# szbonaldo/FedMLP

Measured on AMD Instinct MI355X. Metric: images/sec/client (ICH 224x224 bs=128) at 1/2/4/8 GPUs; mAP vs ref, higher is better.
Workload: dtype f32; 1 GPU; FedMLP stage1 step, Resnet18, ICH-shaped synthetic 3x224x224, C=5, bs=128, one client per GPU, FedAvg all-reduce every 40 steps + once at end; parallelism=clients1, rccl_ranks=1, stream_mode=default: frozen teacher + weight gradients on the engine's side stream, arithmetic=fp32 operands+sums; products as 6 exact bf16 partials on the bf16 matrix pipe

## Files before the change

fedmlp_amd/_lib.py:

```python
import ctypes as C
import os

_HERE = os.path.dirname(os.path.abspath(__file__))
LIB_PATH = os.environ.get("FEDMLP_HIP_LIB") or os.path.join(_HERE, "libfedmlp_hip.so")

FM_MAX_CLASSES = 32
FM_COMM_ID_BYTES = 128


class FmConfig(C.Structure):
    _fields_ = [("model", C.c_int32), ("n_classes", C.c_int32), ("in_h", C.c_int32),
                ("in_w", C.c_int32), ("max_images", C.c_int32), ("reserved", C.c_int32 * 3),
                ("stream", C.c_void_p)]


class FmAdam(C.Structure):
    _fields_ = [("lr", C.c_float), ("beta1", C.c_float), ("beta2", C.c_float),
                ("eps", C.c_float), ("weight_decay", C.c_float)]


class FmSgd(C.Structure):
    _fields_ = [("lr", C.c_float), ("momentum", C.c_float), ("dampening", C.c_float),
                ("weight_decay", C.c_float), ("nesterov", C.c_int32)]

# ... 63 lines not shown
    "fm_profile_read": (C.c_int, [_P, _I32, C.POINTER(_I64), C.POINTER(C.c_double),
                                  C.POINTER(C.c_double)]),
    "fm_comm_preflight": (C.c_int, []),
    "fm_comm_unique_id": (C.c_int, [C.POINTER(C.c_uint8)]),
    "fm_comm_init": (C.c_int, [_P, C.POINTER(C.c_uint8), _I32, _I32]),
    "fm_comm_destroy": (C.c_int, [_P]),
    "fm_comm_size": (C.c_int, [_P]),
    "fm_fedavg_allreduce": (C.c_int, [_P, C.c_float]),
    "fm_fedavg_tao": (C.c_int, [_P, C.POINTER(C.c_double), C.c_double, _F, C.POINTER(C.c_double)]),
    "fm_fedavg_proto": (C.c_int, [_P, _P, C.c_double, _F, _P]),
    "fm_profile_ops": (C.c_int, [_P, _I32, C.c_char_p, _I32]),
    "fm_debug_num_convs": (C.c_int, [_P]),
    "fm_debug_conv_info": (C.c_int, [_P, _I32, C.POINTER(_I32)]),
    "fm_debug_conv": (C.c_int, [_P, _I32, _I32, _P, _P, _P, _I32, _I32, _P]),
    "fm_debug_block_dgrad": (C.c_int, [_P, _I32, _P, _P, _P, _I32]),
    "fm_debug_pw": (C.c_int, [_P, _I32, _I32, _P, _P, _P, _I32, _I32, _P, _P, _P, _P]),
    "fm_debug_proj_bwd": (C.c_int, [_P, _I32, _I32, _P, _P, _P, _P, _P, _I32, _I32, _P, _P]),
    "fm_debug_exp_bwd": (C.c_int, [_P, _I32, _P, _P, _P, _P, _P, _I32, _I32, _P, _P]),
    "fm_debug_get_grads": (C.c_int, [_P, _P]),
    "fm_debug_activation": (C.c_int, [_P, _I32, _I32, _I32, _P, C.POINTER(_I32)]),
    "fm_debug_stem_masks": (C.c_int, [_P, _I32, _I32, _P, _P]),
    "fm_debug_lose_part": (C.c_int, [_I32]),
    "fm_debug_ew": (C.c_int, [_P, _I32, C.POINTER(_P), C.POINTER(_I32), _F]),
    "fm_debug_eff": (C.c_int, [_P, _I32, C.POINTER(_P), C.POINTER(_I32), _F]),
    "fm_debug_eff_ws": (C.c_int, [_I32, C.POINTER(_I32), C.POINTER(C.c_int64)]),
}

_lib = None


# ... 39 lines not shown
```

fedmlp_amd/csrc/common.h:

```cpp
#pragma once
#include <hip/hip_runtime.h>
#include <stdint.h>

#include <stdlib.h>

typedef float f32x4 __attribute__((ext_vector_type(4)));

#ifndef FM_F32_FAST_SWISH
#define FM_F32_FAST_SWISH 1
#endif
#ifdef __HIPCC__
__device__ __forceinline__ float fm_swish_f32(float v)
{
#if FM_F32_FAST_SWISH
    return v * __builtin_amdgcn_rcpf(1.f + __expf(-v));
#else
    return v / (1.f + expf(-v));
#endif
}
#endif


#ifndef FM_MFMA_SPLIT_DEFAULT
#define FM_MFMA_SPLIT_DEFAULT 6
// ... 51 lines not shown
template <int NV> __device__ __forceinline__ void ldf(const float* p, f32x4 (&v)[NV])
{
#pragma unroll
    for (int h = 0; h < NV; ++h) v[h] = ld4(p + 4 * h);
}
#endif

#define PCONV_MAX_JOBS 5
struct PconvJob {
    int ntaps;
    unsigned long long tapcode;
    int cib, icc2;
    unsigned wofs, wofs2;
    int Hg, Wg;
    int oh0, ow0;
    int nsteps, k2;
    int npix;
    float rcpHW, rcpW;
    int tilesN;
    int tile0, step0;
};
inline unsigned long long pconv_tapcode(const int* dh, const int* dw, int ntaps)
{
    unsigned long long c = 0;
    for (int t = 0; t < ntaps; ++t) c |= (unsigned long long)(((dh[t] + 1) & 3) | (((dw[t] + 1) & 3) << 2)) << (4 * t);
    return c;
}

struct IgemmParams {
    const float* W;
// ... 119 lines not shown
```

fedmlp_amd/csrc/engine.hip:

```cpp
#include <math.h>
#include <stdio.h>
#include <string.h>

#include <algorithm>
#include <string>
#include <vector>

#include "../../include/fedmlp_hip.h"
#include "../../include/fedmlp_hip_debug.h"
#include "comm.h"
#include "common.h"
#include "kernels.h"
#include "pwconv.h"

static thread_local std::string g_err;
const char* fm_last_error(void) { return g_err.c_str(); }
const char* fm_version(void) { return "fedmlp_hip 0.2 (gfx950)"; }

#define HIPCHK(x)                                                                              \
    do {                                                                                       \
        hipError_t e_ = (x);                                                                   \
        if (e_ != hipSuccess) {                                                                \
            char b_[512];                                                                      \
            snprintf(b_, sizeof b_, "%s:%d %s -> %s", __FILE__, __LINE__, #x, hipGetErrorString(e_)); \
// ... 144 lines not shown
    size_t off_fcw = 0, off_fcb = 0, off_gamma = 0, off_beta = 0, off_rm = 0, off_rv = 0;
    int64_t nf_sd = 0, ni_sd = 0;
    float *grad = nullptr, *adam_m = nullptr, *adam_v = nullptr;
    float* stage_sd = nullptr;
    fm_adam hp{3e-5f, 0.9f, 0.999f, 1e-8f, 5e-4f};
    int64_t adam_t = 0;
    float *x4 = nullptr, *dyh0 = nullptr;
    float* x3 = nullptr;
    bool stem_rows = false;
    unsigned short* x3p = nullptr;
    long long x3p_plane_elems = 0;
    uint8_t* idx0 = nullptr;
    float *GA = nullptr, *GB = nullptr, *GC = nullptr, *GD = nullptr, *GE = nullptr;
    float *ws_stats = nullptr, *ws_part = nullptr;
    int stats_conv = -1, stats_tiles_n = 0;
    size_t slab_floats = 0;
    float *ca = nullptr, *cb = nullptr, *cc = nullptr;
    float *feat = nullptr, *logits = nullptr, *tfeat = nullptr, *tlogits = nullptr, *dlogits = nullptr;
    float* psum = nullptr;
    int64_t *pcnt = nullptr, *tcnt = nullptr;
    float* zeros = nullptr;
    int *sel_counts = nullptr, *sel_top = nullptr, *sel_bot = nullptr, *cls_dev = nullptr;
    int sel_cap = 0;
    int* tag_buf = nullptr;
    size_t tag_buf_ints = 0;
    bool prof = false, prof_fail = false;
    hipError_t soft_err = hipSuccess;
    int* dev_err = nullptr;
    int* host_err = nullptr;
    int* host_err_dev = nullptr;
// ... 651 lines not shown
    bool side = e->stream_mode != 1;
    const Conv& c0 = e->convs[0];
    if (e->model == 0) {
        const size_t pooled = B * (c0.hout / 2) * (c0.wout / 2) * 64;
        DALLOC(e->idx0, pooled);
        DALLOC(e->dyh0, B * c0.hout * c0.wout * 64);
        DALLOC(e->GA, pooled); DALLOC(e->GB, pooled); DALLOC(e->GC, pooled); DALLOC(e->GD, pooled); DALLOC(e->GE, pooled);
    } else {
        const EffSizes z = eff_sizes(e);
        AALLOC(e->GA, z.g_io); AALLOC(e->GB, z.g_io);
        AALLOC(e->T_small, z.t_small); AALLOC(e->T_big, z.t_big);
        DALLOC(e->se_dgp, B * z.max_ce); DALLOC(e->se_drp, B * z.max_cs); DALLOC(e->se_ds, B * z.max_ce);
        side = side && side_fits(e);
        DALLOC(e->hfeat, B * e->D);
    }
    DALLOC(e->ws_stats, max_stats);
    DALLOC(e->ws_part, (size_t)2 * (1024 + 32) * 2 * e->maxC);
    e->slab_floats = std::max<size_t>(max_slab * 8, (size_t)48 << 20);
    DALLOC(e->main.ws_slab, e->slab_floats);
    e->main.rec = e->main.ws_slab;
    DALLOC(e->ca, 2 * e->maxC); DALLOC(e->cb, 2 * e->maxC); DALLOC(e->cc, 2 * e->maxC);
    DALLOC(e->feat, B * e->D); DALLOC(e->tfeat, B * e->D);
    DALLOC(e->logits, B * e->C); DALLOC(e->tlogits, B * e->C); DALLOC(e->dlogits, B * e->C);
    DALLOC(e->psum, (size_t)2 * e->C * e->D); DALLOC(e->pcnt, 2 * e->C); DALLOC(e->tcnt, e->C);
    DALLOC(e->sel_counts, 2); DALLOC(e->cls_dev, FM_MAX_CLASSES);
    DALLOC(e->zeros, 64);
    if (e->planes) {
        const size_t pooled = B * (c0.hout / 2) * (c0.wout / 2) * 64;
        PALLOC(e->GBp, pooled); PALLOC(e->GCp, pooled); PALLOC(e->GDp, pooled);
        size_t mx = 0;
        for (auto& c : e->convs) {
// ... 87 lines not shown
    if (e->stem_rows && c.stem3) return stem_rows_stats_tiles(imgs_per_group, c.hout);
    if (e->precision && (c.k == 1 || c.cin == 3))
        return pw_blocks(imgs_per_group * c.hout * c.wout, groups, c.cout_p, c.cin == 3 ? c.Kw : c.cin_p, pro_gate, c.hout * c.wout);
    if (conv_uses_pconv(e, c, imgs_per_group * groups)) return (imgs_per_group * c.hout * c.wout + pconv_tile_n(c.cout_p) - 1) / pconv_tile_n(c.cout_p);
    const int bn = igemm_tile_n(c.cout_p, c.cin == 3);
    return (imgs_per_group * c.hout * c.wout + bn - 1) / bn;
}

void conv_fwd(fm_engine* e, Lane& L, int ci, const Weights& W, const float* x, float* y, int imgs, int groups,
              const float* scale, const float* shift, const float* res, int relu, float* stats,
              const Prologue* pro = nullptr, const unsigned short* xp = nullptr, unsigned short* yp = nullptr,
              const unsigned short* resp = nullptr)
{
    Conv& c = e->convs[ci];
    if (stats) {
        e->stats_conv = ci;
        e->stats_tiles_n = stats_tiles_for(e, c, imgs / groups, groups, pro && pro->gate);
    }
    if (e->stem_rows && c.stem3) {
        StemRowsParams q{};
        q.Xp = e->x3p; q.Wst = W.wst; q.Y = y;
        q.scale = scale; q.shift = shift; q.stats = stats; q.relu = relu;
        q.imgs = imgs; q.imgs_per_group = imgs / groups; q.Hp = c.Hp; q.Wp = c.Wp; q.Ho = c.hout; q.Wo = c.wout;
        q.sp = e->products; q.plane_bytes = e->x3p_plane_elems * 2;
        ProfScope ps(e, L, 2, 2.0 * c.macs_per_img * imgs);
        launch_stem_rows(q, L.st);
        return;
    }
    if (conv_uses_pconv(e, c, imgs)) {
        IgemmParams p{};
// ... 57 lines not shown
    if (c.stem3) { p.Hi = c.Hp; p.Wi = c.Wp; }
    p.Hg = c.hout; p.Wg = c.wout; p.sg = c.stride;
    p.Ho = c.hout; p.Wo = c.wout; p.Co = c.cout_p;
    p.os = 1; p.oh0 = 0; p.ow0 = 0;
    p.imgs_per_group = imgs / groups;
    p.tilesM = (c.cout_p + igemm_tile_m(c.cout_p) - 1) / igemm_tile_m(c.cout_p);
    const int bn = igemm_tile_n(c.cout_p, c.cin == 3);
    p.tilesN = (p.imgs_per_group * c.hout * c.wout + bn - 1) / bn;
    p.relu = relu;
    ProfScope ps(e, L, c.cin == 3 ? 2 : (c.cout_p >= 128 ? 0 : 1), 2.0 * c.macs_per_img * imgs);
    launch_igemm(p, groups, L.st);
}

int stats_tiles(fm_engine* e, int ci)
{
    if (e->stats_conv != ci) soft(e, hipErrorInvalidValue);
    return e->stats_tiles_n;
}

void conv_dgrad(fm_engine* e, Lane& L, int ci, const float* dy, float* dx, int imgs, const float* res,
                bool acc_cls0, const unsigned short* dyp = nullptr)
{
    Conv& c = e->convs[ci];
    if (e->planes && c.ncls > 0 && c.cls[0].bm_off >= 0 &&
        pconv_takes(c.cin_p, c.cout_p, (long long)imgs * c.hout * c.wout, c.wout)) {
        const long long xp_pix = (long long)imgs * c.hout * c.wout;
        if (!dyp) dyp = scratch_planes(e, L, dy, xp_pix, c.cout_p);
        for (int k = 0; k < c.ncls; ++k) {
            DgradClass& d = c.cls[k];
            IgemmParams p{};
            p.Xp = dyp; p.xp_pix = xp_pix; p.Wsp = e->wbm_d + d.bm_off;
            p.Y = dx; p.slab = L.sk_slab; p.counters = L.sk_counters; p.err = e->dev_err; p.err_host = e->host_err_dev; p.sp = e->products;
            p.ntaps = d.taps.n;
// ... 94 lines not shown
        PconvJob& j = p.job[k];
        j.ntaps = q.taps.n; j.tapcode = pconv_tapcode(q.dh, q.dw, q.taps.n);
        j.cib = j.icc2 = c.cout_p >> 5;
        j.wofs = j.wofs2 = (unsigned)(q.bm_off * 2);
        j.Hg = (c.hin - q.ph + c.stride - 1) / c.stride;
        j.Wg = (c.win - q.pw + c.stride - 1) / c.stride;
        j.oh0 = q.ph; j.ow0 = q.pw;
    }
    p.job[0].cib += d.cout_p >> 5;
    p.job[0].wofs2 = (unsigned)(d0.bm_off * 2);
    ProfScope ps(e, L, (c.cin_p >= 128 ? 0 : 1) + 6, 2.0 * (c.macs_per_img + d.macs_per_img) * imgs);
    launch_pconv(p, 1, L.st);
    return true;
}

void conv_wgrad(fm_engine* e, Lane& L, int ci, const float* x, const float* dy, int imgs, const Prologue* pro = nullptr,
                int pix_per_group = 0, const unsigned short* xp = nullptr, const unsigned short* dyp = nullptr)
{
    const Conv& c = e->convs[ci];
    if (e->planes && c.cin != 3 &&
        pwgrad_takes(c.cout_p, c.cin_p, c.k, (long long)imgs * c.hout * c.wout, (long long)imgs * c.hin * c.win, c.win, c.pad)) {
        PwgradParams q{};
        q.npix = (long long)imgs * c.hout * c.wout; q.xpix = (long long)imgs * c.hin * c.win;
        if (!xp) xp = scratch_planes(e, L, x, q.xpix, c.cin_p);
        if (!dyp) {
            if ((size_t)q.npix * c.cout_p * 3 > e->xp_scratch_elems) { soft(e, hipErrorInvalidValue); return; }
            k_split_planes(dy, e->xp_scratch2, q.npix, c.cout_p, L.st);
            dyp = e->xp_scratch2;
        }
        q.dYp = dyp; q.Xp = xp; q.slab = L.ws_slab;
// ... 64 lines not shown

void bn_fwd_fixed(fm_engine* e, Lane& L, Bn& b, int groups)
{
    k_bn_finalize_frozen(groups, b.C, e->student.state + e->off_gamma + b.ch_off, e->student.state + e->off_beta + b.ch_off,
                         e->student.state + e->off_rm + b.ch_off, e->student.state + e->off_rv + b.ch_off, b.mean, b.istd, b.scale, b.shift,
                         e->bn_eps, L.st, e->dev_err);
}

void bn_fwd_finalize(fm_engine* e, Lane& L, int ci, int groups, int imgs_per_group, BnMode mode)
{
    const Conv& c = e->convs[ci];
    const int bi = c.bn;
    Bn& b = e->bns[bi];
    if (mode == BnMode::Frozen) { bn_fwd_fixed(e, L, b, groups); return; }
    const bool run = mode == BnMode::Batch;
    k_bn_finalize(e->ws_stats, groups, stats_tiles(e, ci), b.C, imgs_per_group * c.hout * c.wout,
                  e->student.state + e->off_gamma + b.ch_off, e->student.state + e->off_beta + b.ch_off,
                  run ? e->student.state + e->off_rm + b.ch_off : nullptr, run ? e->student.state + e->off_rv + b.ch_off : nullptr, b.mean,
                  b.istd, b.scale, b.shift, e->bn_eps, e->bn_mom, L.st, e->dev_err);
    if (run) e->student.counters[bi] += groups;
}

void bn_bwd(fm_engine* e, Lane& L, int bi, const float* dz, const float* z, float* dy, float* dyh_out, int groups,
            int imgs_per_group, bool frozen, bool z_is_relu_of_bn = false, unsigned short* dyp = nullptr, const unsigned short* zh = nullptr)
{
    const Conv& c = e->convs[bi];
    Bn& b = e->bns[bi];
    const int pix = imgs_per_group * c.hout * c.wout;
    const char* fy = getenv("FM_BN_MASK_FROM_Y");
    const int from_y = fy ? atoi(fy) : 1;
    const float *msc = nullptr, *msh = nullptr;
// ... 43 lines not shown
        if (pm && outp)
            k_bn_apply_planes(y, e->bns[b1].scale, e->bns[b1].shift, res, y2, s2, h2, nullptr, outp, groups, pix, C, 1, L.st, resp);
        else
            k_bn_apply(y, e->bns[b1].scale, e->bns[b1].shift, res, y2, s2, h2, out, groups, pix, C, 1, L.st);
    };
    const float* cur = A.p0;
    const unsigned short* curp = A.p0p;
    bool cur_f32 = true;
    for (size_t bi = 0; bi < e->blocks.size(); ++bi) {
        const Block& blk = e->blocks[bi];
        BlockActs& a = A.blk[bi];
        Conv& c1 = e->convs[blk.c1];
        Conv& c2 = e->convs[blk.c2];
        const int pix = B * c1.hout * c1.wout;
        const bool last = bi + 1 == e->blocks.size();
        conv_fwd(e, L, blk.c1, W, cur, c1.y, imgs, groups, nullptr, nullptr, nullptr, 0, e->ws_stats, nullptr, curp);
        bn_fwd_finalize(e, L, blk.c1, groups, B, mode);
        apply(c1.y, blk.c1, nullptr, nullptr, nullptr, -1, a.z1, a.z1p, pix, c1.cout);
        conv_fwd(e, L, blk.c2, W, a.z1, c2.y, imgs, groups, nullptr, nullptr, nullptr, 0, e->ws_stats, nullptr, a.z1p);
        bn_fwd_finalize(e, L, blk.c2, groups, B, mode);
        unsigned short* outp = (pm && !last) ? a.outp : nullptr;
        if (blk.ds >= 0) {
            Conv& cd = e->convs[blk.ds];
            conv_fwd(e, L, blk.ds, W, cur, cd.y, imgs, groups, nullptr, nullptr, nullptr, 0, e->ws_stats, nullptr, curp);
            bn_fwd_finalize(e, L, blk.ds, groups, B, mode);
            apply(c2.y, blk.c2, nullptr, nullptr, cd.y, blk.ds, a.out, outp, pix, c2.cout);
        } else if (pm && !cur_f32) {
            if (last) {
                k_planes_to_f32(curp, A.blk[bi - 1].out, (long long)imgs * c1.hin * c1.win, c1.cin, L.st);
                apply(c2.y, blk.c2, A.blk[bi - 1].out, nullptr, nullptr, -1, a.out, nullptr, pix, c2.cout);
            } else
                apply(c2.y, blk.c2, nullptr, curp, nullptr, -1, a.out, outp, pix, c2.cout);
        } else {
            apply(c2.y, blk.c2, cur, nullptr, nullptr, -1, a.out, outp, pix, c2.cout);
        }
        cur = a.out;
        curp = a.outp;
        cur_f32 = !(pm && !last);
    }
// ... 13 lines not shown
    }
    auto sc = [&](int bi) { return W.ev_scale + e->bns[bi].ch_off; };
    auto sh = [&](int bi) { return W.ev_shift + e->bns[bi].ch_off; };
    Conv& c0 = e->convs[0];
    conv_fwd(e, L, 0, W, e->x4, A.stem_y, imgs, 1, sc(0), sh(0), nullptr, 1, nullptr);
    const bool pm = e->planes;
    if (pm) k_stem_pool_planes(A.stem_y, nullptr, nullptr, A.p0, nullptr, A.p0p, 1, imgs, c0.hout, c0.wout, 64, L.st);
    else k_stem_pool(A.stem_y, nullptr, nullptr, A.p0, nullptr, 1, imgs, c0.hout, c0.wout, 64, L.st);
    const float* cur = A.p0;
    const unsigned short* curp = A.p0p;
    bool cur_f32 = true;
    for (size_t bi = 0; bi < e->blocks.size(); ++bi) {
        const Block& blk = e->blocks[bi];
        BlockActs& a = A.blk[bi];
        const bool last = bi + 1 == e->blocks.size();
        conv_fwd(e, L, blk.c1, W, cur, pm ? nullptr : a.z1, imgs, 1, sc(blk.c1), sh(blk.c1), nullptr, 1, nullptr, nullptr, curp,
                 pm ? a.z1p : nullptr);
        const float* idt = cur;
        const unsigned short* idtp = nullptr;
        if (blk.ds >= 0) {
            conv_fwd(e, L, blk.ds, W, cur, a.ds_y, imgs, 1, sc(blk.ds), sh(blk.ds), nullptr, 0, nullptr, nullptr, curp);
            idt = a.ds_y;
        } else if (!cur_f32) { idt = nullptr; idtp = curp; }
        const bool planes_only = pm && !last;
        conv_fwd(e, L, blk.c2, W, a.z1, planes_only ? nullptr : a.out, imgs, 1, sc(blk.c2), sh(blk.c2), idt, 1, nullptr, nullptr,
                 a.z1p, planes_only ? a.outp : nullptr, idtp);
        cur = a.out;
        curp = a.outp;
        cur_f32 = !planes_only;
    }
    const Conv& cl = e->convs[e->blocks.back().c2];
    k_avgpool(cur, DT_F32, feat, imgs, cl.hout * cl.wout, 512, L.st);
    k_fc_fwd(feat, S + e->off_fcw, S + e->off_fcb, logits, imgs, 512, e->C, L.st);
}

void ensure_packed(fm_engine* e)
// ... 587 lines not shown
            k_oihw_to_ohwi(src + off, arena + en.eng_off, en.O, en.I, en.KH, en.KW, en.Wpad, en.Ipad, L.st, en.Ostride);
            off += en.n;
        } else if (en.kind == 1) {
            if (!np_only || en.eng_off < e->NP)
                HIPCHK(hipMemcpyAsync(arena + en.eng_off, src + off, en.n * 4, hipMemcpyDeviceToDevice, L.st));
            off += en.n;
        }
    }
    return FM_OK;
}

int debug_fold_stats(fm_engine* e, int ci, int groups, float* stats_dev)
{
    const int tiles = stats_tiles(e, ci), n = 2 * e->convs[ci].cout_p;
    std::vector<float> h((size_t)groups * tiles * n), o((size_t)groups * n, 0.f);
    HIPCHK(hipMemcpyAsync(h.data(), e->ws_stats, h.size() * 4, hipMemcpyDeviceToHost, e->main.st));
    HIPCHK(hipStreamSynchronize(e->main.st));
    for (int g = 0; g < groups; ++g)
        for (int k = 0; k < n; ++k) {
            double sum = 0;
            for (int t = 0; t < tiles; ++t) sum += h[((size_t)g * tiles + t) * n + k];
            o[(size_t)g * n + k] = (float)sum;
        }
    HIPCHK(hipMemcpy(stats_dev, o.data(), o.size() * 4, hipMemcpyHostToDevice));
    return FM_OK;
}

ClassVec to_cv(const float* h, int C)
{
    ClassVec v{};
    for (int i = 0; i < C; ++i) v.v[i] = h[i];
// ... 995 lines not shown
    return FM_OK;
}

int fm_debug_block_dgrad(fm_engine* e, int32_t block, const float* dy1_dev, const float* dyd_dev, float* dx_dev, int32_t imgs)
{
    ARGCHK(e && dy1_dev && dyd_dev && dx_dev, "null tensor");
    ARGCHK(e->model == 0 && !e->precision, "fm_debug_block_dgrad: a precision-0 ResNet-18 engine");
    ARGCHK(block >= 0 && block < (int)e->blocks.size() && e->blocks[block].ds >= 0, "block has no downsample");
    ARGCHK(imgs >= 1 && imgs <= e->maxB, "imgs");
    ensure_packed(e);
    const Block& blk = e->blocks[block];
    if (!block_dgrad(e, e->main, blk.c1, blk.ds, dy1_dev, dyd_dev, dx_dev, imgs)) {
        conv_dgrad(e, e->main, blk.ds, dyd_dev, dx_dev, imgs, nullptr, false);
        conv_dgrad(e, e->main, blk.c1, dy1_dev, dx_dev, imgs, nullptr, true);
    }
    return FM_OK;
}

int fm_debug_conv_info(fm_engine* e, int32_t conv, int32_t* info16)
{
    ARGCHK(e && info16 && conv >= 0 && conv < (int)e->convs.size(), "conv index");
    const Conv& c = e->convs[conv];
    const int v[16] = {c.cin, c.cout, c.k, c.stride, c.pad, c.hin, c.win, c.hout, c.wout, c.cin_p, c.Kw, c.kw_p,
                       c.cout_p, 0, 0, 0};
    memcpy(info16, v, sizeof v);
    return FM_OK;
}

int fm_debug_conv(fm_engine* e, int32_t op, int32_t conv, const float* x_dev, const float* dy_dev, float* out_dev,
                  int32_t imgs, int32_t groups, float* stats_dev)
// ... 267 lines not shown
```

fedmlp_amd/csrc/pconv.hip:

```cpp
#include <stdlib.h>

#include <algorithm>
#include <type_traits>

#include "common.h"
#include "kernels.h"
#include "split3.h"

#if __HIP_DEVICE_COMPILE__
template <int IMM> __device__ __forceinline__ sp_u32x4 pc_lds_read128(unsigned addr)
{
    sp_u32x4 v;
    asm volatile("ds_read_b128 %0, %1 offset:%2" : "=v"(v) : "v"(addr), "n"(IMM));
    return v;
}
__device__ __forceinline__ void pc_divmod(int x, int d, float rcp, int& q, int& r)
{
    q = (int)((float)x * rcp);
    r = x - q * d;
    if (r < 0) { --q; r += d; }
    else if (r >= d) { ++q; r -= d; }
}
template <int CTRL> __device__ __forceinline__ float pc_dpp(float v)
{
// ... 483 lines not shown
                            for (int c = 0; c < FC; ++c)
                                part[q][c] = *reinterpret_cast<const f32x4*>(src + (((r + q) * FC + c) * 512 + tid) * 4);
#pragma unroll
                        for (int q = 0; q < 2; ++q)
#pragma unroll
                            for (int c = 0; c < FC; ++c) acc[r + q][c] += part[q][c];
                    }
                }
            }
        }

        PC_T(5);
        if (do_epilogue) {
        const int mbase = m0 + wm * (16 * FR) + 4 * lg;
        const JobV J = jobv(cur.jb);
        if (p.stats) {
            float* red = fsmem;
#pragma unroll
            for (int r = 0; r < FR; ++r) {
                f32x4 s1 = {0.f, 0.f, 0.f, 0.f}, s2 = {0.f, 0.f, 0.f, 0.f};
#pragma unroll
                for (int c = 0; c < FC; ++c) {
                    s1 += acc[r][c];
                    s2 += acc[r][c] * acc[r][c];
                }
#pragma unroll
                for (int q = 0; q < 4; ++q) {
                    float u = s1[q], v = s2[q];
                    u += pc_dpp<0xB1>(u); v += pc_dpp<0xB1>(v);
                    u += pc_dpp<0x4E>(u); v += pc_dpp<0x4E>(v);
                    u += pc_dpp<0x12C>(u); v += pc_dpp<0x12C>(v);
// ... 1 lines not shown
                    if (li == 0) {
                        const int ml = wm * (16 * FR) + 16 * r + 4 * lg + q;
                        red[(wn * BM + ml) * 2 + 0] = u;
                        red[(wn * BM + ml) * 2 + 1] = v;
                    }
                }
            }
            PC_SYNC_LDS();
            for (int ch = tid; ch < BM; ch += 512) {
                float u = 0.f, v = 0.f;
#pragma unroll
                for (int ww = 0; ww < WN; ++ww) {
                    u += red[(ww * BM + ch) * 2 + 0];
                    v += red[(ww * BM + ch) * 2 + 1];
                }
                float* st = p.stats + (size_t)(grp * J.tilesN + tn) * 2 * p.M;
                st[m0 + ch] = u;
                st[p.M + m0 + ch] = v;
            }
        }
        size_t opix[FC];
        bool ok[FC];
#pragma unroll
        for (int c = 0; c < FC; ++c) {
            const int n = n0 + wn * (16 * FC) + 16 * c + li;
            ok[c] = n < J.npix;
            int img, rem, hg, wg;
            pc_divmod(ok[c] ? n : J.npix - 1, J.HWg, J.rcpHW, img, rem);
            pc_divmod(rem, J.Wg, J.rcpW, hg, wg);
            opix[c] = (size_t)((grp * p.imgs_per_group + img) * p.Ho + hg * p.os + J.oh0) * p.Wo + (wg * p.os + J.ow0);
        }
#pragma unroll
        for (int r = 0; r < FR; r += 2) {
            __builtin_amdgcn_sched_barrier(0);
            const int m = mbase + 16 * r;
            const size_t cb = (size_t)(m0 + wm * (16 * FR) + 16 * r) >> 5;
            f32x4 sc0 = {1.f, 1.f, 1.f, 1.f}, sc1 = sc0, sh0 = {0.f, 0.f, 0.f, 0.f}, sh1 = sh0;
            if (p.scale) {
                sc0 = *reinterpret_cast<const f32x4*>(p.scale + m); sc1 = *reinterpret_cast<const f32x4*>(p.scale + m + 16);
                sh0 = *reinterpret_cast<const f32x4*>(p.shift + m); sh1 = *reinterpret_cast<const f32x4*>(p.shift + m + 16);
            }
#pragma unroll
            for (int c = 0; c < FC; ++c) {
                __builtin_amdgcn_sched_barrier(0);
                const size_t o = opix[c] * p.Co;
                f32x4 v0 = acc[r][c], v1 = acc[r + 1][c];
                if (p.scale) { v0 = v0 * sc0 + sh0; v1 = v1 * sc1 + sh1; }
                if (p.res) {
                    const f32x4 a = *reinterpret_cast<const f32x4*>(p.res + o + m), b = *reinterpret_cast<const f32x4*>(p.res + o + m + 16);
                    v0 += a; v1 += b;
                }
                if (p.resp) {
                    const unsigned char* src = reinterpret_cast<const unsigned char*>(p.resp) + ((cb * 3) * (size_t)p.yp_pix + opix[c]) * 64 + lg * 16;
                    const sp_u32x4 H = *reinterpret_cast<const sp_u32x4*>(src);
                    const sp_u32x4 M = *reinterpret_cast<const sp_u32x4*>(src + (size_t)p.yp_pix * 64);
                    const sp_u32x4 L = *reinterpret_cast<const sp_u32x4*>(src + (size_t)p.yp_pix * 128);
#pragma unroll
                    for (int i = 0; i < 4; ++i) {
                        const float lo = (__builtin_bit_cast(float, H[i] << 16) + __builtin_bit_cast(float, M[i] << 16)) +
                                         __builtin_bit_cast(float, L[i] << 16);
                        const float hi = (__builtin_bit_cast(float, H[i] & 0xffff0000u) + __builtin_bit_cast(float, M[i] & 0xffff0000u)) +
                                         __builtin_bit_cast(float, L[i] & 0xffff0000u);
                        if (i < 2) { v0[2 * i] += lo; v0[2 * i + 1] += hi; }
                        else { v1[2 * (i - 2)] += lo; v1[2 * (i - 2) + 1] += hi; }
                    }
                }
                if (p.relu == 1) {
#pragma unroll
                    for (int q = 0; q < 4; ++q) { v0[q] = fmaxf(v0[q], 0.f); v1[q] = fmaxf(v1[q], 0.f); }
                }
                if (!ok[c]) continue;
                if (p.Y) {
                    *reinterpret_cast<f32x4*>(p.Y + o + m) = v0;
                    *reinterpret_cast<f32x4*>(p.Y + o + m + 16) = v1;
                }
                if (p.Yp) {
                    sp_u32x4 H, M, L;
                    split3(v0, v1, H, M, L);
                    unsigned char* dst = reinterpret_cast<unsigned char*>(p.Yp) + ((cb * 3) * (size_t)p.yp_pix + opix[c]) * 64 + lg * 16;
                    *reinterpret_cast<sp_u32x4*>(dst) = H;
                    *reinterpret_cast<sp_u32x4*>(dst + (size_t)p.yp_pix * 64) = M;
                    *reinterpret_cast<sp_u32x4*>(dst + (size_t)p.yp_pix * 128) = L;
                }
            }
        }
        }
        PC_T(6);
        if (!more) break;
        PC_SYNC_LDS();
        cur = nx;
    }
    if (pend_tile >= 0) {
        asm volatile("s_waitcnt vmcnt(0)" ::: "memory");
        __syncthreads();
// ... 109 lines not shown
        set_max_dyn_lds(reinterpret_cast<const void*>(&pconv_kernel<4, 4, 2, 6>), LDS_L, "pconv_kernel<4, 4, 2, 6>");
        set_max_dyn_lds(reinterpret_cast<const void*>(&pconv_kernel<4, 4, 2, 9>), LDS_L, "pconv_kernel<4, 4, 2, 9>");
        set_max_dyn_lds(reinterpret_cast<const void*>(&pconv_kernel<2, 4, 2, 6>), LDS_S, "pconv_kernel<2, 4, 2, 6>");
        set_max_dyn_lds(reinterpret_cast<const void*>(&pconv_kernel<2, 4, 2, 9>), LDS_S, "pconv_kernel<2, 4, 2, 9>");
        attr_done = true;
    }
    const bool ts = pconv_uses_ts(p);
    p.tapcode = pconv_tapcode(p.dh, p.dw, p.ntaps);
    if (p.njobs == 0) {
        p.njobs = 1;
        PconvJob& j = p.job[0];
        j.ntaps = p.ntaps; j.tapcode = p.tapcode;
        j.cib = j.icc2 = p.Ci >> 5; j.wofs = j.wofs2 = 0;
        j.Hg = p.Hg; j.Wg = p.Wg; j.oh0 = p.oh0; j.ow0 = p.ow0;
    }
    if (!p.Xp2) p.Xp2 = p.Xp;
    long long T = 0;
    p.total_steps = 0; p.nsteps = 0; p.wsp_bytes = 0;
    for (int k = 0; k < p.njobs; ++k) {
        PconvJob& j = p.job[k];
        j.nsteps = j.ntaps * j.cib; j.k2 = j.ntaps * j.icc2;
        j.npix = p.imgs_per_group * j.Hg * j.Wg;
        j.rcpHW = 1.0f / (float)(j.Hg * j.Wg); j.rcpW = 1.0f / (float)j.Wg;
        j.tilesN = (j.npix + 255) / 256;
        j.tile0 = (int)T; j.step0 = (int)p.total_steps;
        T += (long long)p.tilesM * j.tilesN * groups;
        p.total_steps += (long long)p.tilesM * j.tilesN * groups * j.nsteps;
        p.nsteps = std::max(p.nsteps, j.nsteps);
        const long long step_bytes = 3LL * p.M * 64;
        p.wsp_bytes = (unsigned)std::max<long long>(p.wsp_bytes, std::max(j.wofs + j.k2 * step_bytes, j.wofs2 + (j.nsteps - j.k2) * step_bytes));
// ... 67 lines not shown
```

fedmlp_amd/engine.py:

```python
import ctypes as C

import numpy as np
import torch

from . import _lib, spec

MODEL_IDS = {"Resnet18": 0, "Efficient_b0": 1}
PRECISION_IDS = {"fp32": 0, "bf16": 1}
PRODUCT_FORMS = {None: 0, 6: 3, 0: 1, 9: 2}


def _ptr(t):
    if t is None:
        return None
    assert t.is_cuda and t.is_contiguous() and t.dtype in (torch.float32, torch.int32, torch.bfloat16), \
        (t.device, t.dtype, t.is_contiguous())
    return C.c_void_p(t.data_ptr())


class Engine:

    def __init__(self, model, n_classes, in_h, in_w, max_images, device=None, precision="fp32", streams=0, products=None):
        if not torch.cuda.is_available():
            raise RuntimeError("fedmlp_amd.Engine needs a GPU (no CPU fallback)")
# ... 490 lines not shown
        _lib.check(self.lib.fm_debug_activation(self.h, kind, block, imgs, out.ctypes.data_as(C.c_void_p), dims))
        return np.ascontiguousarray(out.transpose(0, 3, 1, 2))

    def debug_num_convs(self):
        return self.lib.fm_debug_num_convs(self.h)

    def debug_conv(self, op, conv, x, dy, out, imgs, groups=1, stats=None):
        self._enqueue()
        _lib.check(self.lib.fm_debug_conv(self.h, op, conv, _ptr(x), _ptr(dy), _ptr(out), imgs, groups,
                                          _ptr(stats)))

    def debug_block_dgrad(self, block, dy1, dyd, dx, imgs):
        self._enqueue()
        _lib.check(self.lib.fm_debug_block_dgrad(self.h, block, _ptr(dy1), _ptr(dyd), _ptr(dx), imgs))

    EW_OPS = ("split_planes", "planes_to_f32", "bn_finalize", "bn_finalize_frozen", "bn_eval_affine", "bn_apply",
              "bn_apply_planes", "stem_pool", "stem_pool_planes", "stem_pool_bwd", "stem_pool_bn_reduce", "stem_pool_bn_apply",
              "bn_bwd_reduce", "bn_bwd_finalize", "bn_bwd_apply", "bn_bwd_apply_planes")

    def debug_ew(self, op, ptrs, dims, scalars=()):
        assert len(ptrs) <= 12 and len(dims) <= 5 and len(scalars) <= 2, (len(ptrs), len(dims), len(scalars))
        for t in ptrs:
            assert t is None or (t.is_cuda and t.is_contiguous()), op
        p = (C.c_void_p * 12)(*[None if t is None else t.data_ptr() for t in ptrs])
        d = (C.c_int32 * 5)(*[int(v) for v in dims])
        _lib.check(self.lib.fm_debug_ew(self.h, self.EW_OPS.index(op), p, d, _lib.fvec(list(scalars) + [0.0] * (2 - len(scalars)))))

    EFF_OPS = ("dw_fwd", "dw_dgrad", "dw_wgrad", "se_fwd", "se_scale", "se_bwd_bn1", "se_wgrad")

    def debug_eff_ws(self, op, dims):
# ... 61 lines not shown
```

include/fedmlp_hip_debug.h:

```cpp
#ifndef FEDMLP_HIP_DEBUG_H
#define FEDMLP_HIP_DEBUG_H

#include "fedmlp_hip.h"

#ifdef __cplusplus
extern "C" {
#endif

int fm_debug_conv_info(fm_engine* e, int32_t conv, int32_t* info16);
int fm_debug_num_convs(fm_engine* e);
int fm_debug_conv(fm_engine* e, int32_t op, int32_t conv, const float* x_dev, const float* dy_dev,
                  float* out_dev, int32_t imgs, int32_t groups, float* stats_dev);

int fm_debug_block_dgrad(fm_engine* e, int32_t block, const float* dy1_dev, const float* dyd_dev, float* dx_dev, int32_t imgs);

int fm_debug_pw(fm_engine* e, int32_t op, int32_t conv, const void* x_dev, const void* dy_dev, void* out_dev,
                int32_t imgs, int32_t groups, const float* psc_dev, const float* psh_dev, const float* gate_dev,
                float* stats_dev);

int fm_debug_proj_bwd(fm_engine* e, int32_t conv, int32_t phase, const void* dyp_dev, const void* yd_dev, const float* bn_dev,
                      const float* gate_dev, const float* ds_dev, int32_t imgs, int32_t groups, void* out_dev,
                      float* pool5_dev);

int fm_debug_exp_bwd(fm_engine* e, int32_t conv, const void* da_dev, const void* ye_dev, const void* x_dev, const void* res_dev,
                     const float* bn_dev, int32_t imgs, int32_t groups, void* dx_dev, float* dw_dev);

int fm_debug_activation(fm_engine* e, int32_t kind, int32_t block, int32_t imgs, float* host_nhwc,
                        int32_t* dims4);

// ... 28 lines not shown
```

Measured before the change: 6081 images/sec.

## Run block conv1 and downsample convs as one grouped implicit-GEMM launch

In ResNet-18 downsampling blocks, the 3x3 stride-2 conv1 and the 1x1 stride-2 downsample conv read the same input, and they now run as two jobs in one pconv launch. Each job gets its own output pointers, BN affine, ReLU flag and stats buffer, and a second stats workspace lets both convs' batch statistics be finalized. The goal is to save a launch, fill the GPU better on the small late-stage layers, and share input planes between the two convs. In exchange, the epilogue carries per-job output state, and the two jobs differ in tap count, which may load-balance poorly.

Result: no change. 6066 images/sec (-0.3%).

```diff
diff --git a/fedmlp_amd/_lib.py b/fedmlp_amd/_lib.py
--- a/fedmlp_amd/_lib.py
+++ b/fedmlp_amd/_lib.py
@@ -101,6 +101,7 @@
     "fm_debug_conv_info": (C.c_int, [_P, _I32, C.POINTER(_I32)]),
     "fm_debug_conv": (C.c_int, [_P, _I32, _I32, _P, _P, _P, _I32, _I32, _P]),
     "fm_debug_block_dgrad": (C.c_int, [_P, _I32, _P, _P, _P, _I32]),
+    "fm_debug_block_fwd": (C.c_int, [_P, _I32, _I32, _P, _P, _P, _I32, _I32, _P, _P, _P]),
     "fm_debug_pw": (C.c_int, [_P, _I32, _I32, _P, _P, _P, _I32, _I32, _P, _P, _P, _P]),
     "fm_debug_proj_bwd": (C.c_int, [_P, _I32, _I32, _P, _P, _P, _P, _P, _I32, _I32, _P, _P]),
     "fm_debug_exp_bwd": (C.c_int, [_P, _I32, _P, _P, _P, _P, _P, _I32, _I32, _P, _P]),
diff --git a/fedmlp_amd/csrc/common.h b/fedmlp_amd/csrc/common.h
--- a/fedmlp_amd/csrc/common.h
+++ b/fedmlp_amd/csrc/common.h
@@ -89,6 +89,13 @@
     unsigned wofs, wofs2;
     int Hg, Wg;
     int oh0, ow0;
+    int own_out;
+    float* Y;
+    unsigned short* Yp;
+    const float* scale;
+    const float* shift;
+    float* stats;
+    int relu;
     int nsteps, k2;
     int npix;
     float rcpHW, rcpW;
diff --git a/fedmlp_amd/csrc/engine.hip b/fedmlp_amd/csrc/engine.hip
--- a/fedmlp_amd/csrc/engine.hip
+++ b/fedmlp_amd/csrc/engine.hip
@@ -182,6 +182,8 @@
     float *GA = nullptr, *GB = nullptr, *GC = nullptr, *GD = nullptr, *GE = nullptr;
     float *ws_stats = nullptr, *ws_part = nullptr;
     int stats_conv = -1, stats_tiles_n = 0;
+    float* ws_stats2 = nullptr;
+    int stats2_conv = -1, stats2_tiles_n = 0;
     size_t slab_floats = 0;
     float *ca = nullptr, *cb = nullptr, *cc = nullptr;
     float *feat = nullptr, *logits = nullptr, *tfeat = nullptr, *tlogits = nullptr, *dlogits = nullptr;
@@ -863,7 +865,8 @@
         side = side && side_fits(e);
         DALLOC(e->hfeat, B * e->D);
     }
-    DALLOC(e->ws_stats, max_stats);
+    DALLOC(e->ws_stats, 2 * max_stats);
+    e->ws_stats2 = e->ws_stats + max_stats;
     DALLOC(e->ws_part, (size_t)2 * (1024 + 32) * 2 * e->maxC);
     e->slab_floats = std::max<size_t>(max_slab * 8, (size_t)48 << 20);
     DALLOC(e->main.ws_slab, e->slab_floats);
@@ -981,6 +984,7 @@
 {
     Conv& c = e->convs[ci];
     if (stats) {
+        if (e->stats2_conv == ci) e->stats2_conv = -1;
         e->stats_conv = ci;
         e->stats_tiles_n = stats_tiles_for(e, c, imgs / groups, groups, pro && pro->gate);
     }
@@ -1068,9 +1072,11 @@
 
 int stats_tiles(fm_engine* e, int ci)
 {
+    if (e->stats2_conv == ci) return e->stats2_tiles_n;
     if (e->stats_conv != ci) soft(e, hipErrorInvalidValue);
     return e->stats_tiles_n;
 }
+float* stats_of(fm_engine* e, int ci) { return e->stats2_conv == ci ? e->ws_stats2 : e->ws_stats; }
 
 void conv_dgrad(fm_engine* e, Lane& L, int ci, const float* dy, float* dx, int imgs, const float* res,
                 bool acc_cls0, const unsigned short* dyp = nullptr)
@@ -1195,6 +1201,60 @@
     return true;
 }
 
+struct ConvOut { float* y; unsigned short* yp; const float* scale; const float* shift; int relu; float* stats; };
+bool block_fwd(fm_engine* e, Lane& L, int c1i, int dsi, const Weights& W, const float* x, const unsigned short* xp, int imgs, int groups,
+               const ConvOut& o1, const ConvOut& od)
+{
+    Conv& c = e->convs[c1i];
+    Conv& d = e->convs[dsi];
+    if (!conv_uses_pconv(e, c, imgs) || !conv_uses_pconv(e, d, imgs)) return false;
+    if (c.k != 3 || c.stride != 2 || c.pad != 1 || d.k != 1 || d.stride != 2 || d.pad != 0 || d.cin_p != c.cin_p || d.cout_p != c.cout_p ||
+        d.hin != c.hin || d.win != c.win || d.hout != c.hout || d.wout != c.wout)
+        return false;
+    static_assert(PCONV_MAX_JOBS >= 2, "conv1 and the downsample");
+    IgemmParams p{};
+    p.xp_pix = (long long)imgs * c.hin * c.win;
+    p.Xp = xp ? xp : scratch_planes(e, L, x, p.xp_pix, c.cin_p);
+    if (!p.Xp) return true;
+    p.Wsp = W.wbm_f;
+    p.yp_pix = (long long)imgs * c.hout * c.wout;
+    p.slab = L.sk_slab; p.counters = L.sk_counters; p.err = e->dev_err; p.err_host = e->host_err_dev; p.sp = e->products;
+    p.M = c.cout_p;
+    p.Hi = c.hin; p.Wi = c.win; p.Ci = c.cin_p;
+    p.Hg = c.hout; p.Wg = c.wout; p.sg = c.stride;
+    p.Ho = c.hout; p.Wo = c.wout; p.Co = c.cout_p;
+    p.os = 1;
+    p.imgs_per_group = imgs / groups;
+    p.tilesM = c.cout_p / pconv_tile_m(c.cout_p);
+    p.tilesN = (p.imgs_per_group * c.hout * c.wout + pconv_tile_n(c.cout_p) - 1) / pconv_tile_n(c.cout_p);
+    p.njobs = 2;
+    const Conv* cv[2] = {&c, &d};
+    const ConvOut* ov[2] = {&o1, &od};
+    for (int k = 0; k < 2; ++k) {
+        const Conv& q = *cv[k];
+        PconvJob& j = p.job[k];
+        int dh[9], dw[9];
+        for (int t = 0; t < q.k * q.k; ++t) { dh[t] = t / q.k - q.pad; dw[t] = t % q.k - q.pad; }
+        j.ntaps = q.k * q.k; j.tapcode = pconv_tapcode(dh, dw, j.ntaps);
+        j.cib = j.icc2 = q.cin_p >> 5;
+        j.wofs = j.wofs2 = (unsigned)(q.bm_off * 2);
+        j.Hg = q.hout; j.Wg = q.wout; j.oh0 = 0; j.ow0 = 0;
+        j.own_out = 1;
+        j.Y = ov[k]->y; j.Yp = ov[k]->yp; j.scale = ov[k]->scale; j.shift = ov[k]->shift; j.stats = ov[k]->stats; j.relu = ov[k]->relu;
+    }
+    if (o1.stats) {
+        if (e->stats2_conv == c1i) e->stats2_conv = -1;
+        e->stats_conv = c1i; e->stats_tiles_n = p.tilesN;
+    }
+    if (od.stats) {
+        if (od.stats == e->ws_stats2) { e->stats2_conv = dsi; e->stats2_tiles_n = p.tilesN; }
+        else { e->stats_conv = dsi; e->stats_tiles_n = p.tilesN; }
+    }
+    ProfScope ps(e, L, (c.cout_p >= 128 ? 0 : 1) + 6, 2.0 * (c.macs_per_img + d.macs_per_img) * imgs);
+    launch_pconv(p, groups, L.st);
+    return true;
+}
+
 void conv_wgrad(fm_engine* e, Lane& L, int ci, const float* x, const float* dy, int imgs, const Prologue* pro = nullptr,
                 int pix_per_group = 0, const unsigned short* xp = nullptr, const unsigned short* dyp = nullptr)
 {
@@ -1289,7 +1349,7 @@
     Bn& b = e->bns[bi];
     if (mode == BnMode::Frozen) { bn_fwd_fixed(e, L, b, groups); return; }
     const bool run = mode == BnMode::Batch;
-    k_bn_finalize(e->ws_stats, groups, stats_tiles(e, ci), b.C, imgs_per_group * c.hout * c.wout,
+    k_bn_finalize(stats_of(e, ci), groups, stats_tiles(e, ci), b.C, imgs_per_group * c.hout * c.wout,
                   e->student.state + e->off_gamma + b.ch_off, e->student.state + e->off_beta + b.ch_off,
                   run ? e->student.state + e->off_rm + b.ch_off : nullptr, run ? e->student.state + e->off_rv + b.ch_off : nullptr, b.mean,
                   b.istd, b.scale, b.shift, e->bn_eps, e->bn_mom, L.st, e->dev_err);
@@ -1363,7 +1423,10 @@
         Conv& c2 = e->convs[blk.c2];
         const int pix = B * c1.hout * c1.wout;
         const bool last = bi + 1 == e->blocks.size();
-        conv_fwd(e, L, blk.c1, W, cur, c1.y, imgs, groups, nullptr, nullptr, nullptr, 0, e->ws_stats, nullptr, curp);
+        const bool grouped = blk.ds >= 0 &&
+            block_fwd(e, L, blk.c1, blk.ds, W, cur, curp, imgs, groups, ConvOut{c1.y, nullptr, nullptr, nullptr, 0, e->ws_stats},
+                      ConvOut{e->convs[blk.ds].y, nullptr, nullptr, nullptr, 0, e->ws_stats2});
+        if (!grouped) conv_fwd(e, L, blk.c1, W, cur, c1.y, imgs, groups, nullptr, nullptr, nullptr, 0, e->ws_stats, nullptr, curp);
         bn_fwd_finalize(e, L, blk.c1, groups, B, mode);
         apply(c1.y, blk.c1, nullptr, nullptr, nullptr, -1, a.z1, a.z1p, pix, c1.cout);
         conv_fwd(e, L, blk.c2, W, a.z1, c2.y, imgs, groups, nullptr, nullptr, nullptr, 0, e->ws_stats, nullptr, a.z1p);
@@ -1371,7 +1434,7 @@
         unsigned short* outp = (pm && !last) ? a.outp : nullptr;
         if (blk.ds >= 0) {
             Conv& cd = e->convs[blk.ds];
-            conv_fwd(e, L, blk.ds, W, cur, cd.y, imgs, groups, nullptr, nullptr, nullptr, 0, e->ws_stats, nullptr, curp);
+            if (!grouped) conv_fwd(e, L, blk.ds, W, cur, cd.y, imgs, groups, nullptr, nullptr, nullptr, 0, e->ws_stats, nullptr, curp);
             bn_fwd_finalize(e, L, blk.ds, groups, B, mode);
             apply(c2.y, blk.c2, nullptr, nullptr, cd.y, blk.ds, a.out, outp, pix, c2.cout);
         } else if (pm && !cur_f32) {
@@ -1415,12 +1478,17 @@
         const Block& blk = e->blocks[bi];
         BlockActs& a = A.blk[bi];
         const bool last = bi + 1 == e->blocks.size();
-        conv_fwd(e, L, blk.c1, W, cur, pm ? nullptr : a.z1, imgs, 1, sc(blk.c1), sh(blk.c1), nullptr, 1, nullptr, nullptr, curp,
-                 pm ? a.z1p : nullptr);
+        const bool grouped = blk.ds >= 0 &&
+            block_fwd(e, L, blk.c1, blk.ds, W, cur, curp, imgs, 1,
+                      ConvOut{pm ? nullptr : a.z1, pm ? a.z1p : nullptr, sc(blk.c1), sh(blk.c1), 1, nullptr},
+                      ConvOut{a.ds_y, nullptr, sc(blk.ds), sh(blk.ds), 0, nullptr});
+        if (!grouped)
+            conv_fwd(e, L, blk.c1, W, cur, pm ? nullptr : a.z1, imgs, 1, sc(blk.c1), sh(blk.c1), nullptr, 1, nullptr, nullptr, curp,
+                     pm ? a.z1p : nullptr);
         const float* idt = cur;
         const unsigned short* idtp = nullptr;
         if (blk.ds >= 0) {
-            conv_fwd(e, L, blk.ds, W, cur, a.ds_y, imgs, 1, sc(blk.ds), sh(blk.ds), nullptr, 0, nullptr, nullptr, curp);
+            if (!grouped) conv_fwd(e, L, blk.ds, W, cur, a.ds_y, imgs, 1, sc(blk.ds), sh(blk.ds), nullptr, 0, nullptr, nullptr, curp);
             idt = a.ds_y;
         } else if (!cur_f32) { idt = nullptr; idtp = curp; }
         const bool planes_only = pm && !last;
@@ -2038,7 +2106,7 @@
 {
     const int tiles = stats_tiles(e, ci), n = 2 * e->convs[ci].cout_p;
     std::vector<float> h((size_t)groups * tiles * n), o((size_t)groups * n, 0.f);
-    HIPCHK(hipMemcpyAsync(h.data(), e->ws_stats, h.size() * 4, hipMemcpyDeviceToHost, e->main.st));
+    HIPCHK(hipMemcpyAsync(h.data(), stats_of(e, ci), h.size() * 4, hipMemcpyDeviceToHost, e->main.st));
     HIPCHK(hipStreamSynchronize(e->main.st));
     for (int g = 0; g < groups; ++g)
         for (int k = 0; k < n; ++k) {
@@ -3064,6 +3132,46 @@
         conv_dgrad(e, e->main, blk.ds, dyd_dev, dx_dev, imgs, nullptr, false);
         conv_dgrad(e, e->main, blk.c1, dy1_dev, dx_dev, imgs, nullptr, true);
     }
+    return FM_OK;
+}
+
+int fm_debug_block_fwd(fm_engine* e, int32_t block, int32_t mode, const float* x_dev, float* y1_dev, float* yd_dev, int32_t imgs,
+                       int32_t groups, float* stats1_dev, float* statsd_dev, const float* affine_dev)
+{
+    ARGCHK(e && x_dev && y1_dev && yd_dev, "null tensor");
+    ARGCHK(e->model == 0 && !e->precision, "fm_debug_block_fwd: a precision-0 ResNet-18 engine");
+    ARGCHK(block >= 0 && block < (int)e->blocks.size() && e->blocks[block].ds >= 0, "block has no downsample");
+    ARGCHK(imgs >= 1 && imgs <= e->maxB && groups >= 1 && imgs % groups == 0, "imgs/groups");
+    ARGCHK(mode == 0 || (mode == 1 && affine_dev && groups == 1 && !stats1_dev && !statsd_dev), "mode");
+    ensure_packed(e);
+    const Block& blk = e->blocks[block];
+    const Conv& c = e->convs[blk.c1];
+    Lane& L = e->main;
+    const int C = c.cout_p;
+    if (mode == 0) {
+        const bool st = stats1_dev || statsd_dev;
+        if (!block_fwd(e, L, blk.c1, blk.ds, e->student, x_dev, nullptr, imgs, groups,
+                       ConvOut{y1_dev, nullptr, nullptr, nullptr, 0, st ? e->ws_stats : nullptr},
+                       ConvOut{yd_dev, nullptr, nullptr, nullptr, 0, st ? e->ws_stats2 : nullptr})) {
+            conv_fwd(e, L, blk.c1, e->student, x_dev, y1_dev, imgs, groups, nullptr, nullptr, nullptr, 0, st ? e->ws_stats : nullptr);
+            if (stats1_dev) RCCHK(debug_fold_stats(e, blk.c1, groups, stats1_dev));
+            conv_fwd(e, L, blk.ds, e->student, x_dev, yd_dev, imgs, groups, nullptr, nullptr, nullptr, 0, st ? e->ws_stats : nullptr);
+            if (statsd_dev) RCCHK(debug_fold_stats(e, blk.ds, groups, statsd_dev));
+            return FM_OK;
+        }
+        if (stats1_dev) RCCHK(debug_fold_stats(e, blk.c1, groups, stats1_dev));
+        if (statsd_dev) RCCHK(debug_fold_stats(e, blk.ds, groups, statsd_dev));
+        return FM_OK;
+    }
+    unsigned short* z1p = e->planes ? e->acts.blk[block].z1p : nullptr;
+    const ConvOut o1{z1p ? nullptr : y1_dev, z1p, affine_dev, affine_dev + C, 1, nullptr};
+    const ConvOut od{yd_dev, nullptr, affine_dev + 2 * C, affine_dev + 3 * C, 0, nullptr};
+    if (!block_fwd(e, L, blk.c1, blk.ds, e->student, x_dev, nullptr, imgs, 1, o1, od)) {
+        conv_fwd(e, L, blk.c1, e->student, x_dev, o1.y, imgs, 1, o1.scale, o1.shift, nullptr, 1, nullptr, nullptr, nullptr, z1p);
+        conv_fwd(e, L, blk.ds, e->student, x_dev, yd_dev, imgs, 1, od.scale, od.shift, nullptr, 0, nullptr);
+    }
+    if (z1p) k_planes_to_f32(z1p, y1_dev, (long long)imgs * c.hout * c.wout, c.cout, L.st);
+    HIPCHK(hipGetLastError());
     return FM_OK;
 }
 
diff --git a/fedmlp_amd/csrc/pconv.hip b/fedmlp_amd/csrc/pconv.hip
--- a/fedmlp_amd/csrc/pconv.hip
+++ b/fedmlp_amd/csrc/pconv.hip
@@ -521,7 +521,14 @@
         if (do_epilogue) {
         const int mbase = m0 + wm * (16 * FR) + 4 * lg;
         const JobV J = jobv(cur.jb);
-        if (p.stats) {
+        struct OutV { float* Y; unsigned short* Yp; const float* scale; const float* shift; float* stats; int relu; };
+        OutV O;
+        if constexpr (TS) O = OutV{p.Y, p.Yp, p.scale, p.shift, p.stats, p.relu};
+        else {
+            const PconvJob& j = p.job[cur.jb];
+            O = OutV{j.Y, j.Yp, j.scale, j.shift, j.stats, j.relu};
+        }
+        if (O.stats) {
             float* red = fsmem;
 #pragma unroll
             for (int r = 0; r < FR; ++r) {
@@ -553,7 +560,7 @@
                     u += red[(ww * BM + ch) * 2 + 0];
                     v += red[(ww * BM + ch) * 2 + 1];
                 }
-                float* st = p.stats + (size_t)(grp * J.tilesN + tn) * 2 * p.M;
+                float* st = O.stats + (size_t)(grp * J.tilesN + tn) * 2 * p.M;
                 st[m0 + ch] = u;
                 st[p.M + m0 + ch] = v;
             }
@@ -575,16 +582,16 @@
             const int m = mbase + 16 * r;
             const size_t cb = (size_t)(m0 + wm * (16 * FR) + 16 * r) >> 5;
             f32x4 sc0 = {1.f, 1.f, 1.f, 1.f}, sc1 = sc0, sh0 = {0.f, 0.f, 0.f, 0.f}, sh1 = sh0;
-            if (p.scale) {
-                sc0 = *reinterpret_cast<const f32x4*>(p.scale + m); sc1 = *reinterpret_cast<const f32x4*>(p.scale + m + 16);
-                sh0 = *reinterpret_cast<const f32x4*>(p.shift + m); sh1 = *reinterpret_cast<const f32x4*>(p.shift + m + 16);
+            if (O.scale) {
+                sc0 = *reinterpret_cast<const f32x4*>(O.scale + m); sc1 = *reinterpret_cast<const f32x4*>(O.scale + m + 16);
+                sh0 = *reinterpret_cast<const f32x4*>(O.shift + m); sh1 = *reinterpret_cast<const f32x4*>(O.shift + m + 16);
             }
 #pragma unroll
             for (int c = 0; c < FC; ++c) {
                 __builtin_amdgcn_sched_barrier(0);
                 const size_t o = opix[c] * p.Co;
                 f32x4 v0 = acc[r][c], v1 = acc[r + 1][c];
-                if (p.scale) { v0 = v0 * sc0 + sh0; v1 = v1 * sc1 + sh1; }
+                if (O.scale) { v0 = v0 * sc0 + sh0; v1 = v1 * sc1 + sh1; }
                 if (p.res) {
                     const f32x4 a = *reinterpret_cast<const f32x4*>(p.res + o + m), b = *reinterpret_cast<const f32x4*>(p.res + o + m + 16);
                     v0 += a; v1 += b;
@@ -604,19 +611,19 @@
                         else { v1[2 * (i - 2)] += lo; v1[2 * (i - 2) + 1] += hi; }
                     }
                 }
-                if (p.relu == 1) {
+                if (O.relu == 1) {
 #pragma unroll
                     for (int q = 0; q < 4; ++q) { v0[q] = fmaxf(v0[q], 0.f); v1[q] = fmaxf(v1[q], 0.f); }
                 }
                 if (!ok[c]) continue;
-                if (p.Y) {
-                    *reinterpret_cast<f32x4*>(p.Y + o + m) = v0;
-                    *reinterpret_cast<f32x4*>(p.Y + o + m + 16) = v1;
-                }
-                if (p.Yp) {
+                if (O.Y) {
+                    *reinterpret_cast<f32x4*>(O.Y + o + m) = v0;
+                    *reinterpret_cast<f32x4*>(O.Y + o + m + 16) = v1;
+                }
+                if (O.Yp) {
                     sp_u32x4 H, M, L;
                     split3(v0, v1, H, M, L);
-                    unsigned char* dst = reinterpret_cast<unsigned char*>(p.Yp) + ((cb * 3) * (size_t)p.yp_pix + opix[c]) * 64 + lg * 16;
+                    unsigned char* dst = reinterpret_cast<unsigned char*>(O.Yp) + ((cb * 3) * (size_t)p.yp_pix + opix[c]) * 64 + lg * 16;
                     *reinterpret_cast<sp_u32x4*>(dst) = H;
                     *reinterpret_cast<sp_u32x4*>(dst + (size_t)p.yp_pix * 64) = M;
                     *reinterpret_cast<sp_u32x4*>(dst + (size_t)p.yp_pix * 128) = L;
@@ -756,6 +763,11 @@
         j.cib = j.icc2 = p.Ci >> 5; j.wofs = j.wofs2 = 0;
         j.Hg = p.Hg; j.Wg = p.Wg; j.oh0 = p.oh0; j.ow0 = p.ow0;
     }
+    for (int k = 0; k < p.njobs; ++k) {
+        PconvJob& j = p.job[k];
+        if (j.own_out) continue;
+        j.Y = p.Y; j.Yp = p.Yp; j.scale = p.scale; j.shift = p.shift; j.stats = p.stats; j.relu = p.relu;
+    }
     if (!p.Xp2) p.Xp2 = p.Xp;
     long long T = 0;
     p.total_steps = 0; p.nsteps = 0; p.wsp_bytes = 0;
diff --git a/fedmlp_amd/engine.py b/fedmlp_amd/engine.py
--- a/fedmlp_amd/engine.py
+++ b/fedmlp_amd/engine.py
@@ -528,6 +528,11 @@
         self._enqueue()
         _lib.check(self.lib.fm_debug_block_dgrad(self.h, block, _ptr(dy1), _ptr(dyd), _ptr(dx), imgs))
 
+    def debug_block_fwd(self, block, mode, x, y1, yd, imgs, groups=1, stats1=None, statsd=None, affine=None):
+        self._enqueue()
+        _lib.check(self.lib.fm_debug_block_fwd(self.h, block, mode, _ptr(x), _ptr(y1), _ptr(yd), imgs, groups, _ptr(stats1),
+                                               _ptr(statsd), _ptr(affine)))
+
     EW_OPS = ("split_planes", "planes_to_f32", "bn_finalize", "bn_finalize_frozen", "bn_eval_affine", "bn_apply",
               "bn_apply_planes", "stem_pool", "stem_pool_planes", "stem_pool_bwd", "stem_pool_bn_reduce", "stem_pool_bn_apply",
               "bn_bwd_reduce", "bn_bwd_finalize", "bn_bwd_apply", "bn_bwd_apply_planes")
diff --git a/include/fedmlp_hip_debug.h b/include/fedmlp_hip_debug.h
--- a/include/fedmlp_hip_debug.h
+++ b/include/fedmlp_hip_debug.h
@@ -13,6 +13,9 @@
                   float* out_dev, int32_t imgs, int32_t groups, float* stats_dev);
 
 int fm_debug_block_dgrad(fm_engine* e, int32_t block, const float* dy1_dev, const float* dyd_dev, float* dx_dev, int32_t imgs);
+
+int fm_debug_block_fwd(fm_engine* e, int32_t block, int32_t mode, const float* x_dev, float* y1_dev, float* yd_dev, int32_t imgs,
+                       int32_t groups, float* stats1_dev, float* statsd_dev, const float* affine_dev);
 
 int fm_debug_pw(fm_engine* e, int32_t op, int32_t conv, const void* x_dev, const void* dy_dev, void* out_dev,
                 int32_t imgs, int32_t groups, const float* psc_dev, const float* psh_dev, const float* gate_dev,
```
